# georgeretsi/smirk

Hardware: AMD Instinct MI355X
Metric: faces/sec (encode+FLAME+render+generate) @224x224 (higher is better)
Workload: dtype f32 results; encoder + generator convs as split-fp16 x3 MFMA with f32 accumulate (fp32-class error), FLAME / raster f32

## Files before the change

include/smirk_hip.h:

```cpp
#ifndef SMIRK_HIP_H
#define SMIRK_HIP_H

#include <stddef.h>
#include <stdint.h>

#ifdef __cplusplus
extern "C" {
#endif

#define SMIRK_OK 0
#define SMIRK_ERR_BAD_ARG (-1)
#define SMIRK_ERR_WORKSPACE (-2)
#define SMIRK_ERR_LAUNCH (-3)
#define SMIRK_ERR_UNSUPPORTED (-4)

const char* smirk_strerror(int code);
unsigned smirk_range_flag_peek(void);
void smirk_range_flag_clear(void);

int smirk_abi_version(void);

#define SMIRK_FLAME_KCHUNK 32

typedef struct SmirkFlameModel {
// ... 21 lines not shown
    const int32_t* dyn_faces;     const float* dyn_bary;
    const int32_t* full_faces;    const float* full_bary;
    const int32_t* mp_faces;      const float* mp_bary;
} SmirkFlameModel;

size_t smirk_flame_workspace_bytes(const SmirkFlameModel* m , int B);

int smirk_flame_forward(const SmirkFlameModel* m, int B,
                        const float* shape, int ns_in, const float* exp, int ne_in,
                        const float* global_pose , const float* neck , const float* jaw ,
                        const float* eye , const float* eyelid ,
                        float* verts, float* lmk_fan, float* lmk_fan3d, float* lmk_mp, int32_t* lut_idx_out,
                        float* v_posed_out, void* ws, size_t ws_bytes, void* stream);

size_t smirk_flame_backward_workspace_bytes(const SmirkFlameModel* m , int B);
int smirk_flame_backward(const SmirkFlameModel* m, const float* dirs_t, int B,
                         const float* shape, int ns_in, const float* exp, int ne_in,
                         const float* global_pose, const float* neck, const float* jaw, const float* eye, const float* eyelid,
                         const float* v_posed, const int32_t* lut_idx,
                         const float* g_verts, const float* g_lmk_fan, const float* g_lmk_fan3d, const float* g_lmk_mp,
                         float* d_shape, float* d_exp, float* d_global_pose, float* d_neck, float* d_jaw, float* d_eye, float* d_eyelid,
                         void* ws, size_t ws_bytes, void* stream);

int smirk_vertices2landmarks(const float* verts, int B, int V, const int32_t* faces ,
                             const int32_t* faces_idx, const float* bary, int L, float* out, void* stream);

typedef struct SmirkRenderMesh {
    int32_t V;
    int32_t Vf;
    int32_t Ff;
    int32_t nnz;
    const int32_t* keep;
    const int32_t* faces;
    const int32_t* nrm_ptr;
    const int32_t* nrm_face;
    const int32_t* nrm_corner;
} SmirkRenderMesh;

size_t smirk_render_workspace_bytes(const SmirkRenderMesh* mesh , int B, int H, int W);

int smirk_render_forward(const SmirkRenderMesh* mesh, int B, int H, int W,
                         const float* verts, const float* cam,
                         float* transformed, float* img,
                         int64_t* pix_to_face, float* bary, float* zbuf, float* normals,
                         void* ws, size_t ws_bytes, void* stream);

int smirk_vertex_normals(const SmirkRenderMesh* mesh, int B, const float* verts, float* normals, void* stream);

int smirk_project_landmarks(const float* lmk, const float* cam, int B, int L, float* out, void* stream);

size_t smirk_render_backward_workspace_bytes(const SmirkRenderMesh* mesh , int B, int H, int W);
int smirk_render_backward(const SmirkRenderMesh* mesh, int B, int H, int W,
                          const float* verts, const float* cam, const int64_t* pix_to_face,
                          const float* g_img, const float* g_transformed,
                          float* d_verts, float* d_cam, void* ws, size_t ws_bytes, void* stream);

int smirk_project_landmarks_backward(const float* lmk, const float* cam, const float* g_out, int B, int L,
                                     float* d_lmk, float* d_cam_accum, void* stream);

enum { SMIRK_PAD_ZERO = 0, SMIRK_PAD_REFLECT = 1 };
enum { SMIRK_ACT_NONE = 0, SMIRK_ACT_RELU = 1 };
enum { SMIRK_OUT_NHWC = 0, SMIRK_OUT_CONVT2X2 = 1 };

typedef struct SmirkConvDesc {
    int32_t B, H, W;
    int32_t C0, C1;
    int32_t Cout;
    int32_t KH, KW;
    int32_t stride;
    int32_t pad_t, pad_l;
    int32_t Ho, Wo;
    int32_t pad_mode;
    int32_t act;
    int32_t out_mode;
} SmirkConvDesc;

int smirk_conv_igemm_f32(const SmirkConvDesc* d, const float* in0, const float* in1, const float* w,
                         const float* scale, const float* shift, const float* residual, float* out, void* stream);

int smirk_conv_igemm_f16x3(const SmirkConvDesc* d, const void* in0, const void* in1, const void* w,
                           const float* scale, const float* shift, const void* residual, void* out, void* stream);
int smirk_conv_igemm_f16x1(const SmirkConvDesc* d, const void* in0, const void* in1, const void* w,
                           const float* scale, const float* shift, const void* residual, void* out, void* stream);
int smirk_conv3x3_tail_f16x3(const SmirkConvDesc* d, const void* in0, const void* in1, const void* w, const float* scale,
                             const float* shift, const float* fw, const float* fb, float* out_nchw, int fcout, void* stream);
int smirk_conv3x3_pool_f16x3(const SmirkConvDesc* d, const void* in0, const void* in1, const void* w, const float* scale, const float* shift, void* out,
                             void* pooled, void* stream);
int smirk_enc1_fused_supported(int cin_pad, int features, int H, int W);
int smirk_enc1_fused_split16(const void* x, const void* w1, const float* scale1, const float* shift1, const void* w2, const float* scale2,
                             const float* shift2, void* e1, void* pooled, int B, int H, int W, void* stream);
int smirk_f32_to_split16(const float* in, void* out, size_t n_elems, void* stream);
int smirk_split16_to_f32(const void* in, float* out, size_t n_elems, void* stream);
int smirk_split16_range_check(const void* in, size_t n_elems, float limit, uint32_t* counts, void* stream);
int smirk_maxpool2x2_split16(const void* in, void* out, int B, int H, int W, int C, void* stream);
int smirk_pack_generator_input_split16(const float* a, int Ca, const float* b, int Cb, void* out, int B, int H, int W, void* stream);
int smirk_conv1x1_sigmoid_nchw_split16(const void* in, const float* w , const float* bias, float* out,
                                       int B, int H, int W, int C, int Cout, void* stream);

int smirk_maxpool2x2_nhwc(const float* in, float* out, int B, int H, int W, int C, void* stream);
int smirk_nchw_to_nhwc_pad(const float* in, float* out, int B, int Cin, int H, int W, int Cpad, void* stream);
int smirk_pack_generator_input(const float* rendered, const float* masked, float* out, int B, int H, int W, void* stream);
int smirk_conv1x1_sigmoid_nchw(const float* in, const float* w , const float* bias, float* out,
                               int B, int H, int W, int C, int Cout, void* stream);

int smirk_stem_conv_s2(const float* img_nchw, const float* w , const float* scale,
                       const float* shift, float* out, int B, int H, int W, int Cout, void* stream);
int smirk_dwconv3x3(const float* in, const float* w , const float* scale, const float* shift, float* out,
                    int B, int H, int W, int C, int stride, int relu, void* stream);
int smirk_gap_linear(const float* feat, const float* w, const float* bias, float* out, float* ws, int B, int HW, int C, int N,
                     void* stream);
int smirk_stem_conv_s2_split16(const float* img_nchw, const float* w, const float* scale, const float* shift, void* out, int B, int H,
                               int W, int Cout, void* stream);
int smirk_dwconv3x3_split16(const void* in, const float* w , const float* scale, const float* shift, void* out, int B, int H,
                            int W, int C, int stride, int relu, void* stream);
int smirk_gap_linear_split16(const void* feat, const float* w, const float* bias, float* out, float* ws, int B, int HW, int C, int N,
                             void* stream);
int smirk_expression_clamps(float* params, int B, int n_exp, void* stream);

int smirk_mask_face_weights(const float* tverts, const float* normals, const int32_t* faces , const float* face_prob ,
                            int B, int V, int F, float* weights , void* stream);
int smirk_sample_faces(const float* weights, int B, int F, int num, uint64_t seed, uint64_t offset, int32_t* idx, float* bary,
                       void* stream);
int smirk_points_to_pixels(const float* points, int B, int L, int image_size, int64_t* out, void* stream);
int smirk_maxpool_sq(const float* in, float* tmp, float* out, int B, int H, int W, int radius, int complement, void* stream);
int smirk_bernoulli_field(float* out, size_t n, float p, uint64_t seed, uint64_t offset, void* stream);
int smirk_masking_compose(const float* img, const float* mask, const float* rendered_mask, const float* extra_points ,
                          const float* pmask ,
                          const float* keep, const float* noise_mult, int B, int C, int H, int W, int gen_noise,
                          uint64_t seed, uint64_t offset, float* out, void* stream);
int smirk_rendered_mask(const float* rendered_img, int B, int C, int H, int W, float* out, void* stream);
int smirk_scatter_points_mask(const int64_t* points, const int64_t* rbound, int B, int L, int H, int W, float* out, void* stream);
int smirk_transfer_pixels(const float* img, const int64_t* points1, const int64_t* points2, const int64_t* rbound, int B, int C,
                          int L, int H, int W, int32_t* winner_ws, float* out, void* stream);

size_t smirk_mbconv_lds_bytes(int Cin, int mid, int Cout, int stride);
int smirk_mbconv_image_supported(int H, int W, int Cin, int mid, int Cout, int stride);
int smirk_mbconv_image_split16(const void* x, const void* wexp, const float* s1, const float* b1, const float* wdw, const float* s2, const float* b2,
                               const void* wproj, const float* s3, const float* b3, int residual, void* out, int B, int H, int W, int Cin, int mid,
                               int Cout, void* stream);
int smirk_encoder_head_supported(int stem_cout, int kind, int cin, int mid, int cout, int stride, int skip);
int smirk_encoder_head_fused_split16(const float* img, const float* stem_w, const float* stem_scale, const float* stem_shift, const float* dw_w,
                                     const float* dw_scale, const float* dw_shift, const void* pw_w, const float* pw_scale, const float* pw_shift,
                                     int residual, void* out, int B, int H, int W, int stride, void* stream);
int smirk_mbconv_supported(int Cin, int mid, int Cout, int stride);
int smirk_mbconv_fused_split16(const void* x, const void* wexp, const float* s1, const float* b1, const float* wdw, const float* s2,
                               const float* b2, const void* wproj, const float* s3, const float* b3, int residual, void* out,
                               int B, int H, int W, int Cin, int mid, int Cout, int stride, void* stream);

typedef struct SmirkConvLayer {
    const void* w;
    const float* scale;
    const float* shift;
} SmirkConvLayer;

#define SMIRK_GEN_MAX_RES 16
enum { SMIRK_PRECISION_F32 = 0, SMIRK_PRECISION_F16X3 = 1 };

typedef struct SmirkGeneratorWeights {
    int32_t in_channels, out_channels, features, res_blocks;
    int32_t precision;
    int32_t cin_pad;
    SmirkConvLayer enc[5][2];
    SmirkConvLayer res[SMIRK_GEN_MAX_RES][2];
    SmirkConvLayer up[4];
    SmirkConvLayer dec[4][2];
    const float* final_w;
// ... 115 lines not shown
```

smirk_amd/_lib.py:

```python
import ctypes as C
import os

import torch

HERE = os.path.dirname(os.path.abspath(__file__))
LIB_PATH = os.path.join(HERE, "lib", "libsmirk_hip.so")
LIB_PATH = os.environ.get("SMIRK_HIP_LIBRARY", LIB_PATH)
ABI_VERSION = 12
PACK_DEPTHWISE, PACK_STEM, PACK_CONVT2X2 = -3, -27, -2
SMIRK_OK, SMIRK_ERR_BAD_ARG, SMIRK_ERR_WORKSPACE, SMIRK_ERR_LAUNCH, SMIRK_ERR_UNSUPPORTED = 0, -1, -2, -3, -4

_p = C.c_void_p
_i = C.c_int
_sz = C.c_size_t


class SmirkFlameModel(C.Structure):
    _fields_ = [(n, C.c_int32) for n in ("V", "VP", "F", "n_shape", "n_exp", "KP", "n_static", "n_dyn", "n_lut",
                                         "n_full", "n_mp", "_pad")] + \
               [(n, _p) for n in ("dirs", "v_template", "lbs_weights", "jdirs", "jtemplate", "l_eyelid", "r_eyelid",
                                  "faces", "static_faces", "static_bary", "dyn_faces", "dyn_bary", "full_faces",
                                  "full_bary", "mp_faces", "mp_bary")]


class SmirkRenderMesh(C.Structure):
    _fields_ = [(n, C.c_int32) for n in ("V", "Vf", "Ff", "nnz")] + \
               [(n, _p) for n in ("keep", "faces", "nrm_ptr", "nrm_face", "nrm_corner")]


class SmirkConvDesc(C.Structure):
    _fields_ = [(n, C.c_int32) for n in ("B", "H", "W", "C0", "C1", "Cout", "KH", "KW", "stride", "pad_t", "pad_l",
                                         "Ho", "Wo", "pad_mode", "act", "out_mode")]


class SmirkConvLayer(C.Structure):
    _fields_ = [("w", _p), ("scale", _p), ("shift", _p)]


GEN_MAX_RES, BACKBONE_MAX_BLOCKS = 16, 24
PRECISION_F32, PRECISION_F16X3 = 0, 1


class SmirkGeneratorWeights(C.Structure):
    _fields_ = [(n, C.c_int32) for n in ("in_channels", "out_channels", "features", "res_blocks", "precision", "cin_pad")] + \
               [("enc", SmirkConvLayer * 2 * 5), ("res", SmirkConvLayer * 2 * GEN_MAX_RES), ("up", SmirkConvLayer * 4),
                ("dec", SmirkConvLayer * 2 * 4), ("final_w", _p), ("final_b", _p)]


class SmirkMbBlock(C.Structure):
    _fields_ = [(n, C.c_int32) for n in ("kind", "stride", "cin", "mid", "cout", "skip")] + \
               [("pw", SmirkConvLayer), ("dw", SmirkConvLayer), ("pwl", SmirkConvLayer)]


class SmirkBackboneWeights(C.Structure):
    _fields_ = [(n, C.c_int32) for n in ("n_blocks", "precision", "n_out", "clamp_n_exp", "stem_cout", "feat_ch")] + \
               [("stem", SmirkConvLayer), ("blocks", SmirkMbBlock * BACKBONE_MAX_BLOCKS), ("head_w", _p), ("head_b", _p)]


class SmirkProfileRecord(C.Structure):
    _fields_ = [("kernel", C.c_char * 120), ("flop", C.c_double), ("bytes", C.c_double), ("ms", C.c_float), ("_pad", C.c_int32)]


PAD_ZERO, PAD_REFLECT = 0, 1
ACT_NONE, ACT_RELU = 0, 1
OUT_NHWC, OUT_CONVT2X2 = 0, 1

_SIGS = {
    "smirk_strerror": (C.c_char_p, [_i]),
    "smirk_abi_version": (_i, []),
    "smirk_range_flag_peek": (C.c_uint, []),
    "smirk_range_flag_clear": (None, []),
    "smirk_flame_workspace_bytes": (_sz, [C.POINTER(SmirkFlameModel), _i]),
    "smirk_flame_forward": (_i, [C.POINTER(SmirkFlameModel), _i, _p, _i, _p, _i, _p, _p, _p, _p, _p, _p, _p, _p, _p, _p,
                                 _p, _p, _sz, _p]),
    "smirk_flame_backward_workspace_bytes": (_sz, [C.POINTER(SmirkFlameModel), _i]),
    "smirk_flame_backward": (_i, [C.POINTER(SmirkFlameModel), _p, _i, _p, _i, _p, _i] + [_p] * 5 + [_p, _p] + [_p] * 4 + [_p] * 7 +
                             [_p, _sz, _p]),
    "smirk_vertices2landmarks": (_i, [_p, _i, _i, _p, _p, _p, _i, _p, _p]),
    "smirk_render_workspace_bytes": (_sz, [C.POINTER(SmirkRenderMesh), _i, _i, _i]),
    "smirk_render_forward": (_i, [C.POINTER(SmirkRenderMesh), _i, _i, _i, _p, _p, _p, _p, _p, _p, _p, _p, _p, _sz, _p]),
    "smirk_vertex_normals": (_i, [C.POINTER(SmirkRenderMesh), _i, _p, _p, _p]),
    "smirk_mask_face_weights": (_i, [_p, _p, _p, _p, _i, _i, _i, _p, _p]),
    "smirk_sample_faces": (_i, [_p, _i, _i, _i, C.c_uint64, C.c_uint64, _p, _p, _p]),
    "smirk_points_to_pixels": (_i, [_p, _i, _i, _i, _p, _p]),
    "smirk_maxpool_sq": (_i, [_p, _p, _p, _i, _i, _i, _i, _i, _p]),
    "smirk_bernoulli_field": (_i, [_p, _sz, C.c_float, C.c_uint64, C.c_uint64, _p]),
    "smirk_masking_compose": (_i, [_p, _p, _p, _p, _p, _p, _p, _i, _i, _i, _i, _i, C.c_uint64, C.c_uint64, _p, _p]),
    "smirk_render_backward_workspace_bytes": (_sz, [C.POINTER(SmirkRenderMesh), _i, _i, _i]),
    "smirk_render_backward": (_i, [C.POINTER(SmirkRenderMesh), _i, _i, _i, _p, _p, _p, _p, _p, _p, _p, _p, _sz, _p]),
    "smirk_project_landmarks_backward": (_i, [_p, _p, _p, _i, _i, _p, _p, _p]),
    "smirk_encoder_head_supported": (_i, [_i] * 7),
    "smirk_encoder_head_fused_split16": (_i, [_p] * 10 + [_i, _p] + [_i] * 4 + [_p]),
    "smirk_mbconv_image_supported": (_i, [_i] * 6),
    "smirk_mbconv_image_split16": (_i, [_p] * 10 + [_i, _p] + [_i] * 6 + [_p]),
    "smirk_mbconv_lds_bytes": (_sz, [_i, _i, _i, _i]),
    "smirk_mbconv_supported": (_i, [_i, _i, _i, _i]),
    "smirk_mbconv_fused_split16": (_i, [_p] * 10 + [_i, _p] + [_i] * 7 + [_p]),
    "smirk_warp_affine_u8": (_i, [_p, _i, _i, _i, _p, _i, _i, _i, _p, _p, _p]),
    "smirk_resize_linear_u8": (_i, [_p, _i, _i, _i, _i, _i, _i, _p, _p, _p]),
    "smirk_f32_nchw_to_u8_grid": (_i, [_p, _i, _i, _i, _i, _p, _i, _i, _p]),
    "smirk_u8_hwc_to_f32_nchw": (_i, [_p, _i, _i, _i, _i, _p, _p]),
    "smirk_interp_bilinear_f32": (_i, [_p, _i, _i, _i, _i, _i, _p, _p]),
    "smirk_hull_mask": (_i, [_p, _i, _i, _i, _i, _i, _p, _p]),
    "smirk_rendered_mask": (_i, [_p, _i, _i, _i, _i, _p, _p]),
    "smirk_scatter_points_mask": (_i, [_p, _p, _i, _i, _i, _i, _p, _p]),
    "smirk_transfer_pixels": (_i, [_p, _p, _p, _p, _i, _i, _i, _i, _i, _p, _p, _p]),
    "smirk_project_landmarks": (_i, [_p, _p, _i, _i, _p, _p]),
    "smirk_conv_igemm_f32": (_i, [C.POINTER(SmirkConvDesc), _p, _p, _p, _p, _p, _p, _p, _p]),
    "smirk_conv_igemm_f16x3": (_i, [C.POINTER(SmirkConvDesc), _p, _p, _p, _p, _p, _p, _p, _p]),
    "smirk_conv_igemm_f16x1": (_i, [C.POINTER(SmirkConvDesc), _p, _p, _p, _p, _p, _p, _p, _p]),
    "smirk_conv3x3_tail_f16x3": (_i, [C.POINTER(SmirkConvDesc), _p, _p, _p, _p, _p, _p, _p, _p, _i, _p]),
    "smirk_conv3x3_pool_f16x3": (_i, [C.POINTER(SmirkConvDesc), _p, _p, _p, _p, _p, _p, _p, _p]),
    "smirk_enc1_fused_supported": (_i, [_i, _i, _i, _i]),
    "smirk_enc1_fused_split16": (_i, [_p] * 9 + [_i, _i, _i, _p]),
    "smirk_f32_to_split16": (_i, [_p, _p, _sz, _p]),
    "smirk_split16_to_f32": (_i, [_p, _p, _sz, _p]),
    "smirk_maxpool2x2_split16": (_i, [_p, _p, _i, _i, _i, _i, _p]),
    "smirk_split16_range_check": (_i, [_p, _sz, C.c_float, _p, _p]),
    "smirk_pack_generator_input_split16": (_i, [_p, _i, _p, _i, _p, _i, _i, _i, _p]),
    "smirk_conv1x1_sigmoid_nchw_split16": (_i, [_p, _p, _p, _p, _i, _i, _i, _i, _i, _p]),
    "smirk_maxpool2x2_nhwc": (_i, [_p, _p, _i, _i, _i, _i, _p]),
    "smirk_nchw_to_nhwc_pad": (_i, [_p, _p, _i, _i, _i, _i, _i, _p]),
    "smirk_pack_generator_input": (_i, [_p, _p, _p, _i, _i, _i, _p]),
    "smirk_conv1x1_sigmoid_nchw": (_i, [_p, _p, _p, _p, _i, _i, _i, _i, _i, _p]),
    "smirk_stem_conv_s2": (_i, [_p, _p, _p, _p, _p, _i, _i, _i, _i, _p]),
    "smirk_dwconv3x3": (_i, [_p, _p, _p, _p, _p, _i, _i, _i, _i, _i, _i, _p]),
    "smirk_gap_linear": (_i, [_p, _p, _p, _p, _p, _i, _i, _i, _i, _p]),
    "smirk_stem_conv_s2_split16": (_i, [_p, _p, _p, _p, _p, _i, _i, _i, _i, _p]),
    "smirk_dwconv3x3_split16": (_i, [_p, _p, _p, _p, _p, _i, _i, _i, _i, _i, _i, _p]),
    "smirk_gap_linear_split16": (_i, [_p, _p, _p, _p, _p, _i, _i, _i, _i, _p]),
    "smirk_expression_clamps": (_i, [_p, _i, _i, _p]),
    "smirk_generator_workspace_bytes": (_sz, [C.POINTER(SmirkGeneratorWeights), _i, _i, _i]),
    "smirk_generator_forward": (_i, [C.POINTER(SmirkGeneratorWeights), _p, _i, _p, _i, _p, _i, _i, _i, C.POINTER(_p), _p, _sz, _p]),
    "smirk_backbone_workspace_bytes": (_sz, [C.POINTER(SmirkBackboneWeights), _i, _i, _i]),
    "smirk_backbone_forward": (_i, [C.POINTER(SmirkBackboneWeights), _p, _i, _i, _i, _p, _p, _p, _sz, _p]),
    "smirk_train_reduce_workspace_bytes": (_sz, [_i]),
    "smirk_conv_stats_rows_max": (_sz, [C.POINTER(SmirkConvDesc)]),
    "smirk_conv_igemm_stats_split16": (_i, [C.POINTER(SmirkConvDesc), _p, _p, _p, _p, _p, C.POINTER(C.c_int), _i, _p]),
    "smirk_bn_train_forward_partials_split16": (_i, [_p, _sz, _i, _p, _p, _p, _i, C.c_float, C.c_float, _p, _p, _p, _p, _p, _p, _p, _p, _i, _i, _p]),
    "smirk_dwconv3x3_stats_split16": (_i, [_p, _p, _p, _i, _i, _i, _i, _i, _p, C.POINTER(C.c_int), _p]),
    "smirk_bn_train_forward_split16": (_i, [_p, _sz, _i, _p, _p, _p, _i, C.c_float, C.c_float, _p, _p, _p, _p, _p, _p, _p, _p, _sz, _p]),
    "smirk_bn_train_backward_split16": (_i, [_p, _p, _sz, _i, _p, _p, _p, _p, _i, _p, _p, _p, _p, _sz, _p]),
    "smirk_bn_eval_forward_split16": (_i, [_p, _sz, _i, _p, _p, _p, _p, _p, _i, C.c_float, _p, _p, _p, _p]),
    "smirk_bn_eval_backward_split16": (_i, [_p, _p, _sz, _i, _p, _p, _p, _p, _p, _i, _p, _p]),
    "smirk_colsum_split16": (_i, [_p, _sz, _i, _p, _p, _sz, _p]),
    "smirk_maxpool2x2_backward_split16": (_i, [_p, _p, _p, _p, _i, _i, _i, _i, _p]),
    "smirk_reflect_pad1_backward_split16": (_i, [_p, _p, _p, _i, _i, _i, _i, _p]),
    "smirk_space_to_depth2_split16": (_i, [_p, _p, _i, _i, _i, _i, _p]),
    "smirk_conv1x1_sigmoid_backward_split16": (_i, [_p, _p, _p, _p, _p, _i, _i, _i, _i, _i, _p]),
    "smirk_conv_wgrad_set_mode": (_i, [_i]),
    "smirk_conv_wgrad_workspace_bytes": (_sz, [_i, _i, _i, _i, _i, _i]),
    "smirk_conv_wgrad_f32": (_i, [_p, _p, _p, _i, _i, _i, _i, _i, _i, _i, _p, _sz, _p]),
    "smirk_conv_wgrad_f16x1": (_i, [_p, _p, _p, _i, _i, _i, _i, _i, _i, _i, _p, _sz, _p]),
    "smirk_conv_wgrad_param": (_i, [_p, _p, _p, _i, _i, _i, _i, _i, _i, _i, _i, _i, _i, _i, _i, _p, _sz, _p]),
    "smirk_conv_wgrad_x1_fallbacks": (C.c_ulonglong, []),
    "smirk_pack_conv_weights_batch_split16": (_i, [_p, _i, C.c_ulonglong, _p]),
    "smirk_pack_conv_weights_split16": (_i, [_p, _i, _i, _i, _i, _i, _i, _p, _p, _p]),
    "smirk_stem_conv_s2_raw_split16": (_i, [_p, _p, _p, _i, _i, _i, _i, _p]),
    "smirk_stem_conv_s2_wgrad_workspace_bytes": (_sz, [_i]),
    "smirk_stem_conv_s2_wgrad_split16": (_i, [_p, _p, _p, _i, _i, _i, _i, _p, _sz, _p]),
    "smirk_stem_conv_s2_dgrad_split16": (_i, [_p, _p, _p, _i, _i, _i, _i, _p]),
    "smirk_dwconv3x3_dgrad_split16": (_i, [_p, _p, _p, _p, _i, _i, _i, _i, _i, _p]),
    "smirk_dwconv3x3_wgrad_workspace_bytes": (_sz, [_i]),
    "smirk_dwconv3x3_wgrad_split16": (_i, [_p, _p, _p, _i, _i, _i, _i, _i, _p, _sz, _p]),
    "smirk_dwconv3x3_wgrad_param_split16": (_i, [_p, _p, _p, _i, _i, _i, _i, _i, _p, _sz, _p]),
    "smirk_gap_linear_backward_split16": (_i, [_p, _p, _p, _p, _p, _p, _i, _i, _i, _i, _p]),
    "smirk_profile_start": (_i, []),
    "smirk_profile_stop": (_i, [C.POINTER(SmirkProfileRecord), _i]),
    "smirk_random_point_budget": (_i, [_p, _i, _i, C.c_float, C.c_uint64, C.c_uint64, _p]),
    "smirk_cycle_augment_workspace_bytes": (_sz, [_i]),
    "smirk_cycle_augment": (_i, [_p] * 6 + [_i] * 6 + [_p, _p, _p, _i, C.c_uint64, C.c_uint64] + [_p] * 6 + [_p, _p, _sz, _p]),
}
EXPORTS = tuple(_SIGS)

_LIB = None


class SmirkHipError(RuntimeError):
    pass


def lib():
    global _LIB
    if _LIB is None:
        if not os.path.exists(LIB_PATH):
            raise SmirkHipError(f"{LIB_PATH} not found: build it with `python -m smirk_amd.build` "
                                "(smirk_amd has no CPU / eager fallback)")
        L = C.CDLL(LIB_PATH)
        for name, (res, args) in _SIGS.items():
            fn = getattr(L, name)
            fn.restype, fn.argtypes = res, args
        if L.smirk_abi_version() != ABI_VERSION:
            raise SmirkHipError("libsmirk_hip.so ABI version mismatch; rebuild")
# ... 103 lines not shown
```

smirk_amd/csrc/capi.hip:

```cpp
#include <stdlib.h>
#include <string.h>

#include <map>
#include <mutex>
#include <utility>
#include <vector>

#include "common.h"

extern "C" const char* smirk_strerror(int code) {
    switch (code) {
        case SMIRK_OK: return "ok";
        case SMIRK_ERR_BAD_ARG: return "bad argument (null pointer, size or alignment constraint violated)";
        case SMIRK_ERR_WORKSPACE: return "workspace too small (see smirk_*_workspace_bytes)";
        case SMIRK_ERR_LAUNCH: return "HIP kernel launch failed";
        case SMIRK_ERR_UNSUPPORTED: return "configuration not supported by the gfx950 kernels";
        default: return "unknown smirk error";
    }
}

extern "C" int smirk_abi_version(void) { return 12; }

int smirk_switch(SmirkSwitch s) {
    static const char* const names[] = {"SMIRK_IGEMM_HALO", "SMIRK_IGEMM_PP", "SMIRK_CONV_RING", "SMIRK_DISABLE_PATCH_KERNEL", "SMIRK_DISABLE_ENC1_FUSED",
                                        "SMIRK_DISABLE_MBCONV_IMAGE", "SMIRK_DISABLE_MBCONV_TILE", "SMIRK_DISABLE_MBCONV_FUSED",
                                        "SMIRK_DISABLE_ENCODER_HEAD_FUSED", "SMIRK_GEN_SPLIT_CHAINS", "SMIRK_WGRAD_F16"};
    static_assert(sizeof(names) / sizeof(names[0]) == SMIRK_SW_COUNT, "one name per SmirkSwitch");
    const char* e = getenv(names[s]);
    switch (s) {
        case SMIRK_SW_IGEMM_HALO:
        case SMIRK_SW_CONV_RING: return !e || e[0] != '0';
        case SMIRK_SW_IGEMM_PP: return !e ? 1 : e[0] == '0' ? 0 : e[0] == 'a' ? 2 : 1;
        case SMIRK_SW_GEN_SPLIT_CHAINS: return !e ? 0 : e[0] == '0' ? 1 : e[0] == '3' ? 3 : 2;
        case SMIRK_SW_WGRAD_F16: return e ? atoi(e) : SMIRK_WGRAD_F16_DEFAULT;
        default: return e != nullptr;
    }
}

namespace {
std::mutex g_dev_mu;
std::map<std::pair<int, const void*>, size_t> g_lds_raised;
std::map<int, int> g_dev_cus;
}

int smirk_raise_dynamic_lds(const void* kernel, size_t bytes) {
    int dev = 0;
    if (hipGetDevice(&dev) != hipSuccess) { (void)hipGetLastError(); return SMIRK_ERR_LAUNCH; }
    std::lock_guard<std::mutex> lk(g_dev_mu);
    size_t& raised = g_lds_raised[{dev, kernel}];
    if (bytes <= raised) return SMIRK_OK;
    if (hipFuncSetAttribute(kernel, hipFuncAttributeMaxDynamicSharedMemorySize, (int)bytes) != hipSuccess) { (void)hipGetLastError(); return SMIRK_ERR_LAUNCH; }
    raised = bytes;
    return SMIRK_OK;
}

int smirk_device_cus() {
    int dev = 0;
    if (hipGetDevice(&dev) != hipSuccess) { (void)hipGetLastError(); return 256; }
    std::lock_guard<std::mutex> lk(g_dev_mu);
    auto it = g_dev_cus.find(dev);
    if (it != g_dev_cus.end()) return it->second;
    int cus = 0;
    if (hipDeviceGetAttribute(&cus, hipDeviceAttributeMultiprocessorCount, dev) != hipSuccess || cus <= 0) { (void)hipGetLastError(); cus = 256; }
    g_dev_cus[dev] = cus;
    return cus;
}

namespace {
std::once_flag g_range_once;
unsigned* g_range_host = nullptr;
unsigned* g_range_dev = nullptr;
}
unsigned* smirk_range_flag_device_ptr() {
    std::call_once(g_range_once, [] {
        void* h = nullptr;
        if (hipHostMalloc(&h, 64, hipHostMallocMapped | hipHostMallocPortable) != hipSuccess || !h) { (void)hipGetLastError(); return; }
        *(volatile unsigned*)h = 0u;
        void* d = nullptr;
        if (hipHostGetDevicePointer(&d, h, 0) != hipSuccess || !d) { (void)hipGetLastError(); (void)hipHostFree(h); return; }
        g_range_host = (unsigned*)h;
        g_range_dev = (unsigned*)d;
    });
    return g_range_dev;
}
extern "C" unsigned smirk_range_flag_peek(void) { return g_range_host ? *(volatile unsigned*)g_range_host : 0u; }
extern "C" void smirk_range_flag_clear(void) { if (g_range_host) *(volatile unsigned*)g_range_host = 0u; }

bool g_smirk_prof_on = false;
namespace {
struct ProfRec { char name[120]; double flop, bytes; hipEvent_t e0, e1; };
std::vector<ProfRec> g_recs;
std::mutex g_prof_mu;
thread_local char t_next_name[120];
thread_local double t_next_flop = 0.0, t_next_bytes = 0.0;
thread_local bool t_has_name = false;
thread_local long t_open = -1;
}

void smirk_prof_next(const char* name, double flop, double bytes) {
    if (!g_smirk_prof_on) return;
    t_has_name = name != nullptr;
    if (name) { strncpy(t_next_name, name, sizeof(t_next_name) - 1); t_next_name[sizeof(t_next_name) - 1] = 0; }
    t_next_flop = flop; t_next_bytes = bytes;
}
// ... 55 lines not shown
```

smirk_amd/csrc/conv.hip:

```cpp
#include <stdio.h>
#include <stdlib.h>

#include "common.h"
#include <type_traits>

#include "conv_common.h"

__device__ __attribute__((aligned(16))) float g_zero16_conv[4] = {0.f, 0.f, 0.f, 0.f};
#define g_zero16 g_zero16_conv

__device__ __forceinline__ const float* psel(bool c, const float* p, const float* q) {
    const unsigned long long m = 0ull - (unsigned long long)c;
    return (const float*)(((unsigned long long)p & m) | ((unsigned long long)q & ~m));
}

enum { KW_GENERIC = 0, KW_FAST = 1, KW_FAST_KT = 2, KW_CMAJOR = 3, KW_LEAN = 4, KW_LEAN_CM = 5 };

template <int BM, int BN, int WGM, int WGN, bool SPLIT, int KWALK, bool X1 = false, bool STATS = false>
__device__ __forceinline__ void conv_tile(const ConvArgs& a, float* smem, const int m0, const int n0) {
    constexpr int NW = WGM * WGN, NT = 64 * NW;
    constexpr int RP = NT / 8;
    constexpr int TM = BM / WGM / 32, TN = BN / WGN / 32;
    constexpr int PA = BM / RP, PB = BN / RP;
    constexpr int STAGE = (BM + BN) * 32;
// ... 480 lines not shown
                    float v = acc[0][i][j][r] * sc + sh;
                    size_t o;
                    int b, y, x;
                    row_to_pixel(m, HoWo, d.Wo, a.psh, b, y, x);
                    if (convt) o = (((size_t)b * 2 * d.Ho + 2 * y + dy) * 2 * d.Wo + 2 * x + dx) * d.Cout + co;
                    else o = (((size_t)b * d.Ho + y) * d.Wo + x) * d.Cout + n;
                    if (a.residual) v += a.residual[o];
                    if (d.act == SMIRK_ACT_RELU) v = fmaxf(v, 0.f);
                    a.out[o] = v;
                }
            }
        }
    }
}

template <int BM, int BN, int WGM, int WGN, bool SPLIT, int KWALK, bool X1 = false, bool STATS = false>
__global__ __launch_bounds__(64 * WGM * WGN, 2) void conv_igemm_kernel(ConvArgs a) {
    __shared__ __attribute__((aligned(16))) float smem[2 * (BM + BN) * 32];
    const int ntn = (a.N + BN - 1) / BN;
    const int logical = xcd_logical(blockIdx.x, gridDim.x);
    const int mt = logical / ntn, nt = logical % ntn;
    conv_tile<BM, BN, WGM, WGN, SPLIT, KWALK, X1, STATS>(a, smem, mt * BM, nt * BN);
}

template <int BM, int BN, int WGM, int WGN, bool SPLIT, int KWALK, bool X1 = false>
static void launch_igemm_kw(const ConvArgs& a, hipStream_t st) {
    const int ntm = (a.M + BM - 1) / BM, ntn = (a.N + BN - 1) / BN;
    if (g_smirk_prof_on) {
        char nm[120];
        snprintf(nm, sizeof(nm), "conv_igemm_kernel<%d,%d,%d,%d,%s,%d>%s", BM, BN, WGM, WGN, SPLIT ? "true" : "false", KWALK, X1 ? "[f16x1]" : "");
        const double px = (double)a.d.B * a.d.H * a.d.W;
        smirk_prof_next(nm, 2.0 * a.M * a.N * a.K, 4.0 * (px * a.Cin + (double)a.M * a.N + (double)a.N * a.K + (a.residual ? (double)a.M * a.N : 0.0)));
    }
    if constexpr (SPLIT && (KWALK == KW_LEAN || KWALK == KW_LEAN_CM || KWALK == KW_FAST_KT)) {
        if (a.stats) {
            SMIRK_LAUNCH((conv_igemm_kernel<BM, BN, WGM, WGN, SPLIT, KWALK, X1, true>), dim3(ntm * ntn), dim3(64 * WGM * WGN), 0, st, a);
            return;
        }
    }
    SMIRK_LAUNCH((conv_igemm_kernel<BM, BN, WGM, WGN, SPLIT, KWALK, X1>), dim3(ntm * ntn), dim3(64 * WGM * WGN), 0, st, a);
}

template <int BM, int BN, int WGM, int WGN, bool SPLIT, bool X1 = false>
static void launch_igemm(const ConvArgs& a, hipStream_t st) {
    const SmirkConvDesc& d = a.d;
    const bool lean = true;
    if constexpr (SPLIT && WGM * WGN == 4) {
        const long long b0 = (long long)d.B * d.H * d.W * d.C0 * 4, b1 = (long long)d.B * d.H * d.W * d.C1 * 4, bw = (long long)a.N * a.K * 4;
        if (lean && (d.C0 % CV_BK == 0) && (d.C1 % CV_BK == 0) && b0 < (1ll << 31) && b1 < (1ll << 31) && bw < (1ll << 31)) {
            const bool pow2 = (d.C0 & (d.C0 - 1)) == 0 && (d.C1 & (d.C1 - 1)) == 0, even = ((d.C0 + d.C1) / CV_BK) % 2 == 0;
            const bool want_cm = BN == 128;
            if (want_cm && d.KH == 3 && d.KW == 3 && pow2 && even) launch_igemm_kw<BM, BN, WGM, WGN, SPLIT, KW_LEAN_CM, X1>(a, st);
            else launch_igemm_kw<BM, BN, WGM, WGN, SPLIT, KW_LEAN, X1>(a, st);
            return;
        }
    }
    const bool cmajor = BN == 128 && d.Ho * d.Wo >= 400;
    if constexpr (SPLIT && WGM * WGN == 4) {
        if (cmajor && d.KH == 3 && d.KW == 3 && (d.C0 % CV_BK == 0) && (d.C1 % CV_BK == 0)) {
            launch_igemm_kw<BM, BN, WGM, WGN, SPLIT, KW_CMAJOR, X1>(a, st);
            return;
        }
    }
    if ((d.C0 % CV_BK == 0) && (d.C1 % CV_BK == 0)) launch_igemm_kw<BM, BN, WGM, WGN, SPLIT, KW_FAST, X1>(a, st);
    else if (d.KH * d.KW == 1) launch_igemm_kw<BM, BN, WGM, WGN, SPLIT, KW_FAST_KT, X1>(a, st);
    else launch_igemm_kw<BM, BN, WGM, WGN, SPLIT, KW_GENERIC, X1>(a, st);
}

bool smirk_conv_pp_eligible(const ConvArgs& a);
int smirk_conv_pp_launch(const ConvArgs& a, hipStream_t st);

bool smirk_conv_halo_eligible(const ConvArgs& a);
int smirk_conv_halo_launch(const ConvArgs& a, hipStream_t st, bool x1);

bool smirk_conv3x3_patch_eligible(const SmirkConvDesc* d, bool has_residual);
int smirk_conv3x3_patch_launch(const SmirkConvDesc* d, const void* in0, const void* in1, const void* w, const float* scale,
                               const float* shift, void* out, hipStream_t st, const float* fw, const float* fb, float* fout,
                               int fcout);

bool smirk_conv3x3_ring64_eligible(const SmirkConvDesc* d, bool has_residual);
int smirk_conv3x3_ring64_launch(const SmirkConvDesc* d, const void* in0, const void* in1, const void* w, const float* scale, const float* shift, void* out,
                                void* pooled, hipStream_t st, float* stats = nullptr, int* stats_rows = nullptr);

static int conv_dispatch_one(const SmirkConvDesc* d, const void* in0, const void* in1, const void* w, const float* scale,
                             const float* shift, const void* residual, void* out, void* stream, bool split, bool x1 = false, float* stats = nullptr,
                             int* stats_rows = nullptr);

static int conv_batch_chunk(const SmirkConvDesc* d, bool split) {
    if (!split || d->B <= 1) return d->B;
    const long long px = (long long)d->H * d->W, per = 4 * px * (d->C0 > d->C1 ? d->C0 : d->C1), lim = (1ll << 31) - 1;
    if (per * d->B <= lim || per > lim) return d->B;
    return (int)(lim / per);
}

static int conv_dispatch(const SmirkConvDesc* d, const void* in0, const void* in1, const void* w, const float* scale,
                         const float* shift, const void* residual, void* out, void* stream, bool split, bool x1 = false, float* stats = nullptr,
                         int* stats_rows = nullptr) {
    if (!d || !in0 || !w || !out) return SMIRK_ERR_BAD_ARG;
    if (stats_rows) *stats_rows = 0;
    const int bc = (d->B > 0 && d->H > 0 && d->W > 0 && d->C0 > 0 && d->C1 >= 0) ? conv_batch_chunk(d, split) : d->B;
    if (bc >= d->B) return conv_dispatch_one(d, in0, in1, w, scale, shift, residual, out, stream, split, x1, stats, stats_rows);
    const size_t ipx = (size_t)d->H * d->W, opx = (size_t)d->Ho * d->Wo * (d->out_mode == SMIRK_OUT_CONVT2X2 ? 4 : 1);
    for (int b0 = 0; b0 < d->B; b0 += bc) {
        SmirkConvDesc dc = *d;
        dc.B = d->B - b0 < bc ? d->B - b0 : bc;
        const int rc = conv_dispatch_one(&dc, (const float*)in0 + b0 * ipx * d->C0, in1 ? (const float*)in1 + b0 * ipx * d->C1 : nullptr, w, scale, shift,
                                         residual ? (const float*)residual + b0 * opx * d->Cout : nullptr, (float*)out + b0 * opx * d->Cout, stream, split, x1);
        if (rc != SMIRK_OK) return rc;
    }
    return SMIRK_OK;
}

static int conv_dispatch_one(const SmirkConvDesc* d, const void* in0, const void* in1, const void* w, const float* scale,
                             const float* shift, const void* residual, void* out, void* stream, bool split, bool x1, float* stats, int* stats_rows) {
    if (!d || !in0 || !w || !out) return SMIRK_ERR_BAD_ARG;
    if (stats_rows) *stats_rows = 0;
    if (x1 && !split) return SMIRK_ERR_BAD_ARG;
    const int cq = split ? 8 : 4;
    if (d->B <= 0 || d->H <= 0 || d->W <= 0 || d->Cout <= 0 || d->C0 <= 0 || d->C0 % cq || d->C1 % cq || d->C1 < 0 ||
        (d->C1 > 0 && !in1) || d->Ho <= 0 || d->Wo <= 0 || d->stride <= 0 || (split && d->Cout % 8))
        return SMIRK_ERR_BAD_ARG;
    if (!((d->KH == 3 && d->KW == 3) || (d->KH == 1 && d->KW == 1))) return SMIRK_ERR_UNSUPPORTED;
    if (d->pad_mode == SMIRK_PAD_REFLECT && (d->H < 2 || d->W < 2 || d->pad_t > 1 || d->pad_l > 1)) return SMIRK_ERR_UNSUPPORTED;
    ConvArgs a;
    a.d = *d; a.in0 = (const float*)in0; a.in1 = (const float*)in1; a.w = (const float*)w; a.scale = scale; a.shift = shift;
    a.residual = (const float*)residual; a.out = (float*)out;
    a.Cin = d->C0 + d->C1;
    a.K = d->KH * d->KW * a.Cin;
    a.N = d->Cout;
    if (d->out_mode == SMIRK_OUT_CONVT2X2) {
        if (d->KH != 1 || d->C1 != 0 || d->Ho != d->H || d->Wo != d->W || d->stride != 1 || residual) return SMIRK_ERR_UNSUPPORTED;
        a.N = 4 * d->Cout;
    }
    const long long M = (long long)d->B * d->Ho * d->Wo;
    if (M > (1ll << 30) || (long long)d->B * d->H * d->W > (1ll << 30)) return SMIRK_ERR_UNSUPPORTED;
    a.M = (int)M;
    a.stats = nullptr;
    a.psh = 0;
    if (d->KH == 3)
        while (a.psh < 4 && d->Ho % (2 << a.psh) == 0 && d->Wo % (2 << a.psh) == 0) ++a.psh;
    hipStream_t st = (hipStream_t)stream;
    const bool no_patch = smirk_switch(SMIRK_SW_DISABLE_PATCH_KERNEL);
    if (split && !x1 && !no_patch && smirk_conv3x3_ring64_eligible(d, residual != nullptr))
        return smirk_conv3x3_ring64_launch(d, in0, in1, w, scale, shift, out, nullptr, st, stats, stats_rows);
    if (split && !x1 && !no_patch && smirk_conv3x3_patch_eligible(d, residual != nullptr))
        return smirk_conv3x3_patch_launch(d, in0, in1, w, scale, shift, out, st, nullptr, nullptr, nullptr, 0);
    const bool want_stats = split && stats && stats_rows && d->out_mode == SMIRK_OUT_NHWC && !scale && !shift && !residual && d->act == SMIRK_ACT_NONE;
    if (split && smirk_conv_halo_eligible(a)) {
        if (want_stats) { a.stats = stats; *stats_rows = ((a.M + 255) / 256) * 4; }
        return smirk_conv_halo_launch(a, st, x1);
    }
    if (split && !x1 && smirk_conv_pp_eligible(a)) return smirk_conv_pp_launch(a, st);
    if (want_stats) {
        const long long b0 = (long long)d->B * d->H * d->W * d->C0 * 4, b1 = (long long)d->B * d->H * d->W * d->C1 * 4, bw = (long long)a.N * a.K * 4;
        const bool lean = (d->C0 % CV_BK == 0) && (d->C1 % CV_BK == 0) && b0 < (1ll << 31) && b1 < (1ll << 31) && bw < (1ll << 31);
        const bool kt = !((d->C0 % CV_BK == 0) && (d->C1 % CV_BK == 0)) && d->KH * d->KW == 1;
        if (lean || kt) {
            const int BMt = a.N > 32 ? 128 : 256, WGMt = a.N > 32 ? 2 : 4;
            a.stats = stats;
            *stats_rows = ((a.M + BMt - 1) / BMt) * WGMt;
        }
    }
    if (split && x1) {
        if (a.N > 64) launch_igemm<128, 128, 2, 2, true, true>(a, st);
        else if (a.N > 32) launch_igemm<128, 64, 2, 2, true, true>(a, st);
        else launch_igemm<256, 32, 4, 1, true, true>(a, st);
    } else if (split) {
        if (a.N > 64) launch_igemm<128, 128, 2, 2, true>(a, st);
        else if (a.N > 32) launch_igemm<128, 64, 2, 2, true>(a, st);
        else launch_igemm<256, 32, 4, 1, true>(a, st);
    } else {
        if (a.N > 64) launch_igemm<128, 128, 2, 2, false>(a, st);
        else if (a.N > 32) launch_igemm<128, 64, 2, 2, false>(a, st);
        else launch_igemm<256, 32, 4, 1, false>(a, st);
    }
    return smirk_launch_status();
}

extern "C" int smirk_conv_igemm_f32(const SmirkConvDesc* d, const float* in0, const float* in1, const float* w,
                                    const float* scale, const float* shift, const float* residual, float* out,
                                    void* stream) {
    return conv_dispatch(d, in0, in1, w, scale, shift, residual, out, stream, false);
}

extern "C" int smirk_conv3x3_pool_f16x3(const SmirkConvDesc* d, const void* in0, const void* in1, const void* w, const float* scale, const float* shift, void* out,
                                        void* pooled, void* stream) {
    if (!d || !in0 || !w || !out || !pooled) return SMIRK_ERR_BAD_ARG;
    if (d->C0 % 8 || d->C1 % 8 || (d->C1 > 0 && !in1) || d->H % 2 || d->W % 2) return SMIRK_ERR_BAD_ARG;
    if (d->B <= 0 || d->H <= 0 || d->W <= 0 || d->C0 <= 0) return SMIRK_ERR_BAD_ARG;
    const int bc = conv_batch_chunk(d, true);
    if (bc <= 0) return SMIRK_ERR_UNSUPPORTED;
    {
        SmirkConvDesc d0 = *d;
        d0.B = d->B < bc ? d->B : bc;
        if (d0.Cout != 64 || !smirk_conv3x3_ring64_eligible(&d0, false)) return SMIRK_ERR_UNSUPPORTED;
    }
    const size_t px = (size_t)d->H * d->W;
    for (int b0 = 0; b0 < d->B; b0 += bc) {
        SmirkConvDesc dc = *d;
        dc.B = d->B - b0 < bc ? d->B - b0 : bc;
        const int rc = smirk_conv3x3_ring64_launch(&dc, (const float*)in0 + b0 * px * d->C0, in1 ? (const float*)in1 + b0 * px * d->C1 : nullptr, w, scale, shift,
                                                   (float*)out + b0 * px * d->Cout, (float*)pooled + b0 * (px / 4) * d->Cout, (hipStream_t)stream);
        if (rc != SMIRK_OK) return rc;
    }
    return SMIRK_OK;
}

extern "C" int smirk_conv3x3_tail_f16x3(const SmirkConvDesc* d, const void* in0, const void* in1, const void* w, const float* scale,
                                        const float* shift, const float* fw, const float* fb, float* out_nchw, int fcout,
                                        void* stream) {
    if (!d || !in0 || !w || !fw || !out_nchw || fcout <= 0 || fcout > 4 || d->Cout != 32) return SMIRK_ERR_BAD_ARG;
    if (d->C0 % 8 || d->C1 % 8 || (d->C1 > 0 && !in1) || d->act != SMIRK_ACT_RELU) return SMIRK_ERR_BAD_ARG;
    if (!smirk_conv3x3_patch_eligible(d, false)) return SMIRK_ERR_UNSUPPORTED;
    const int bc = (d->B > 0 && d->H > 0 && d->W > 0 && d->C0 > 0 && d->C1 >= 0) ? conv_batch_chunk(d, true) : d->B;
    if (bc >= d->B) return smirk_conv3x3_patch_launch(d, in0, in1, w, scale, shift, nullptr, (hipStream_t)stream, fw, fb, out_nchw, fcout);
    const size_t px = (size_t)d->H * d->W;
    for (int b0 = 0; b0 < d->B; b0 += bc) {
        SmirkConvDesc dc = *d;
        dc.B = d->B - b0 < bc ? d->B - b0 : bc;
        const int rc = smirk_conv3x3_patch_launch(&dc, (const float*)in0 + b0 * px * d->C0, in1 ? (const float*)in1 + b0 * px * d->C1 : nullptr, w, scale, shift,
                                                  nullptr, (hipStream_t)stream, fw, fb, out_nchw + b0 * px * fcout, fcout);
        if (rc != SMIRK_OK) return rc;
    }
    return SMIRK_OK;
}

extern "C" int smirk_conv_igemm_f16x3(const SmirkConvDesc* d, const void* in0, const void* in1, const void* w,
                                      const float* scale, const float* shift, const void* residual, void* out,
                                      void* stream) {
    return conv_dispatch(d, in0, in1, w, scale, shift, residual, out, stream, true);
}

extern "C" int smirk_conv_igemm_f16x1(const SmirkConvDesc* d, const void* in0, const void* in1, const void* w,
                                      const float* scale, const float* shift, const void* residual, void* out,
                                      void* stream) {
// ... 285 lines not shown
```

Before: 10370.

## Add streaming 1x1 conv kernel for small-Cin wide-Cout expansions

Adds a dedicated 1x1 convolution kernel that stages a 64-row activation tile in LDS once and streams over all output-channel tiles, reading weights directly from global memory and computing the split-fp16 products with 32x32x16 MFMA. It is dispatched for NHWC 1x1 convs with C0<=64, Cout>=6*C0 and small spatial maps, targeting expansion convs where the generic igemm tiling wastes work or launches poorly. The per-tile accumulator goes through an LDS transpose buffer for a coalesced epilogue with scale/shift/relu. It adds a new code path whose behaviour under the split precision scheme must match the existing kernels.

```diff
diff --git a/include/smirk_hip.h b/include/smirk_hip.h
--- a/include/smirk_hip.h
+++ b/include/smirk_hip.h
@@ -127,6 +127,7 @@
                            const float* scale, const float* shift, const void* residual, void* out, void* stream);
 int smirk_conv_igemm_f16x1(const SmirkConvDesc* d, const void* in0, const void* in1, const void* w,
                            const float* scale, const float* shift, const void* residual, void* out, void* stream);
+int smirk_conv1x1_stream_eligible(const SmirkConvDesc* d, int has_residual);
 int smirk_conv3x3_tail_f16x3(const SmirkConvDesc* d, const void* in0, const void* in1, const void* w, const float* scale,
                              const float* shift, const float* fw, const float* fb, float* out_nchw, int fcout, void* stream);
 int smirk_conv3x3_pool_f16x3(const SmirkConvDesc* d, const void* in0, const void* in1, const void* w, const float* scale, const float* shift, void* out,
diff --git a/smirk_amd/_lib.py b/smirk_amd/_lib.py
--- a/smirk_amd/_lib.py
+++ b/smirk_amd/_lib.py
@@ -6,7 +6,7 @@
 HERE = os.path.dirname(os.path.abspath(__file__))
 LIB_PATH = os.path.join(HERE, "lib", "libsmirk_hip.so")
 LIB_PATH = os.environ.get("SMIRK_HIP_LIBRARY", LIB_PATH)
-ABI_VERSION = 12
+ABI_VERSION = 13
 PACK_DEPTHWISE, PACK_STEM, PACK_CONVT2X2 = -3, -27, -2
 SMIRK_OK, SMIRK_ERR_BAD_ARG, SMIRK_ERR_WORKSPACE, SMIRK_ERR_LAUNCH, SMIRK_ERR_UNSUPPORTED = 0, -1, -2, -3, -4
 
@@ -109,6 +109,7 @@
     "smirk_conv_igemm_f32": (_i, [C.POINTER(SmirkConvDesc), _p, _p, _p, _p, _p, _p, _p, _p]),
     "smirk_conv_igemm_f16x3": (_i, [C.POINTER(SmirkConvDesc), _p, _p, _p, _p, _p, _p, _p, _p]),
     "smirk_conv_igemm_f16x1": (_i, [C.POINTER(SmirkConvDesc), _p, _p, _p, _p, _p, _p, _p, _p]),
+    "smirk_conv1x1_stream_eligible": (_i, [C.POINTER(SmirkConvDesc), _i]),
     "smirk_conv3x3_tail_f16x3": (_i, [C.POINTER(SmirkConvDesc), _p, _p, _p, _p, _p, _p, _p, _p, _i, _p]),
     "smirk_conv3x3_pool_f16x3": (_i, [C.POINTER(SmirkConvDesc), _p, _p, _p, _p, _p, _p, _p, _p]),
     "smirk_enc1_fused_supported": (_i, [_i, _i, _i, _i]),
diff --git a/smirk_amd/csrc/capi.hip b/smirk_amd/csrc/capi.hip
--- a/smirk_amd/csrc/capi.hip
+++ b/smirk_amd/csrc/capi.hip
@@ -19,7 +19,7 @@
     }
 }
 
-extern "C" int smirk_abi_version(void) { return 12; }
+extern "C" int smirk_abi_version(void) { return 13; }
 
 int smirk_switch(SmirkSwitch s) {
     static const char* const names[] = {"SMIRK_IGEMM_HALO", "SMIRK_IGEMM_PP", "SMIRK_CONV_RING", "SMIRK_DISABLE_PATCH_KERNEL", "SMIRK_DISABLE_ENC1_FUSED",
diff --git a/smirk_amd/csrc/conv.hip b/smirk_amd/csrc/conv.hip
--- a/smirk_amd/csrc/conv.hip
+++ b/smirk_amd/csrc/conv.hip
@@ -586,6 +586,9 @@
 int smirk_conv3x3_ring64_launch(const SmirkConvDesc* d, const void* in0, const void* in1, const void* w, const float* scale, const float* shift, void* out,
                                 void* pooled, hipStream_t st, float* stats = nullptr, int* stats_rows = nullptr);
 
+extern "C" int smirk_conv1x1_stream_eligible(const SmirkConvDesc* d, int has_residual);
+int smirk_conv1x1_stream_launch(const ConvArgs& a, hipStream_t st);
+
 static int conv_dispatch_one(const SmirkConvDesc* d, const void* in0, const void* in1, const void* w, const float* scale,
                              const float* shift, const void* residual, void* out, void* stream, bool split, bool x1 = false, float* stats = nullptr,
                              int* stats_rows = nullptr);
@@ -655,6 +658,7 @@
         return smirk_conv_halo_launch(a, st, x1);
     }
     if (split && !x1 && smirk_conv_pp_eligible(a)) return smirk_conv_pp_launch(a, st);
+    if (split && !x1 && !stats && !no_patch && smirk_conv1x1_stream_eligible(d, residual != nullptr)) return smirk_conv1x1_stream_launch(a, st);
     if (want_stats) {
         const long long b0 = (long long)d->B * d->H * d->W * d->C0 * 4, b1 = (long long)d->B * d->H * d->W * d->C1 * 4, bw = (long long)a.N * a.K * 4;
         const bool lean = (d->C0 % CV_BK == 0) && (d->C1 % CV_BK == 0) && b0 < (1ll << 31) && b1 < (1ll << 31) && bw < (1ll << 31);
diff --git a/smirk_amd/csrc/conv_stream1x1.hip b/smirk_amd/csrc/conv_stream1x1.hip
--- /dev/null
+++ b/smirk_amd/csrc/conv_stream1x1.hip
@@ -0,0 +1,183 @@
+#include <stdio.h>
+
+#include "common.h"
+#include "conv_common.h"
+
+struct S1Args {
+    const float *in, *w, *scale, *shift;
+    float* out;
+    int M, N, K, Cout, H, W;
+    int ksteps, pitch;
+    int convt, relu;
+};
+
+#define S1_ROWS 64
+#define S1_TB (32 * 36)
+
+template <int KG, int NW>
+__global__ __launch_bounds__(64 * NW, KG <= 2 ? 3 : 2) void conv1x1_stream_kernel(S1Args a) {
+    constexpr int NT = 64 * NW;
+    extern __shared__ __attribute__((aligned(16))) char smem[];
+    const int tid = threadIdx.x, lane = tid & 63, fr = lane & 31, hb = lane >> 5;
+    const int wave = __builtin_amdgcn_readfirstlane(tid >> 6);
+    char* As = smem;
+    float* tb = (float*)(smem + S1_ROWS * a.pitch) + wave * S1_TB;
+    const int m0 = blockIdx.x * S1_ROWS;
+    const int nunits = 2 * ((a.N + 31) / 32);
+    const half8 hz = {0, 0, 0, 0, 0, 0, 0, 0};
+
+    auto load_b = [&](int u, int j, half8 (*dst)[2]) {
+        const int n = (u >> 1) * 32 + fr;
+        const bool nv = u < nunits && n < a.N;
+        const float* wrow = a.w + (size_t)(nv ? n : 0) * a.K;
+#pragma unroll
+        for (int s = 0; s < 4; ++s) {
+            const int g = 2 * (4 * j + s) + hb, gc = min(g, a.K / 8 - 1);
+            const bool v = nv && g * 8 < a.K;
+            const half8 t0 = *(const half8*)(wrow + gc * 8), t1 = *(const half8*)(wrow + gc * 8 + 4);
+            dst[s][0] = v ? t0 : hz;
+            dst[s][1] = v ? t1 : hz;
+        }
+    };
+    half8 bn[4][2];
+    load_b(wave, 0, bn);
+
+    {
+        constexpr int NIT = S1_ROWS * KG * 16 / NT;
+        const int P = a.ksteps * 4, Preal = a.K / 4;
+        f32x4 xv[NIT];
+#pragma unroll
+        for (int it = 0; it < NIT; ++it) {
+            const int idx = tid + NT * it, row = idx / P, pc = idx - row * P;
+            const bool in = idx < S1_ROWS * P && m0 + row < a.M && pc < Preal;
+            const f32x4 t = *(const f32x4*)(a.in + (size_t)min(m0 + row, a.M - 1) * a.K + min(pc, Preal - 1) * 4);
+            const f32x4 z = {0.f, 0.f, 0.f, 0.f};
+            xv[it] = in ? t : z;
+        }
+#pragma unroll
+        for (int it = 0; it < NIT; ++it) {
+            const int idx = tid + NT * it, row = idx / P, pc = idx - row * P;
+            if (idx < S1_ROWS * P) *(f32x4*)(As + row * a.pitch + pc * 16) = xv[it];
+        }
+    }
+    asm volatile("s_waitcnt lgkmcnt(0)" ::: "memory");
+    __builtin_amdgcn_s_barrier();
+    asm volatile("" ::: "memory");
+
+    SmirkRangeAcc rng;
+    const int HW = a.H * a.W;
+    for (int u = wave; u < nunits; u += NW) {
+        const int rb = u & 1, n0 = (u >> 1) * 32;
+        const int ng = n0 + (lane & 3) * 8;
+        const bool gv = ng < a.N;
+        const int co = a.convt ? ng % a.Cout : ng, coc = gv ? co : 0;
+        f32x4 sc0 = {1.f, 1.f, 1.f, 1.f}, sc1 = sc0, sh0 = {0.f, 0.f, 0.f, 0.f}, sh1 = sh0;
+        if (a.scale) { sc0 = *(const f32x4*)(a.scale + coc); sc1 = *(const f32x4*)(a.scale + coc + 4); }
+        if (a.shift) { sh0 = *(const f32x4*)(a.shift + coc); sh1 = *(const f32x4*)(a.shift + coc + 4); }
+
+        f32x16 acc0, acc1;
+#pragma unroll
+        for (int r = 0; r < 16; ++r) { acc0[r] = 0.f; acc1[r] = 0.f; }
+        const char* arow = As + (rb * 32 + fr) * a.pitch + hb * 32;
+#pragma unroll
+        for (int j = 0; j < KG; ++j) {
+            half8 bc[4][2];
+#pragma unroll
+            for (int s = 0; s < 4; ++s) { bc[s][0] = bn[s][0]; bc[s][1] = bn[s][1]; }
+            if (j + 1 < KG) load_b(u, j + 1, bn); else load_b(u + NW, 0, bn);
+#pragma unroll
+            for (int s = 0; s < 4; ++s) {
+                const int S = 4 * j + s;
+                if (S < a.ksteps) {
+                    const half8 ah = *(const half8*)(arow + S * 64), al = *(const half8*)(arow + S * 64 + 16);
+                    acc0 = __builtin_amdgcn_mfma_f32_32x32x16_f16(ah, bc[s][0], acc0, 0, 0, 0);
+                    acc1 = __builtin_amdgcn_mfma_f32_32x32x16_f16(ah, bc[s][1], acc1, 0, 0, 0);
+                    acc1 = __builtin_amdgcn_mfma_f32_32x32x16_f16(al, bc[s][0], acc1, 0, 0, 0);
+                }
+            }
+        }
+
+#pragma unroll
+        for (int r = 0; r < 16; ++r) tb[mfma32_row(r, lane) * 36 + fr] = __builtin_fmaf(acc1[r], 1.0f / 2048.0f, acc0[r]);
+        asm volatile("s_waitcnt lgkmcnt(0)" ::: "memory");
+#pragma unroll
+        for (int it = 0; it < 2; ++it) {
+            const int row = (it * 64 + lane) >> 2, m = m0 + rb * 32 + row;
+            if (m < a.M && gv) {
+                float v[8];
+                *(f32x4*)v = *(const f32x4*)(tb + row * 36 + (lane & 3) * 8);
+                *(f32x4*)(v + 4) = *(const f32x4*)(tb + row * 36 + (lane & 3) * 8 + 4);
+                size_t o;
+                if (a.convt) {
+                    const int b = m / HW, rem = m - b * HW, y = rem / a.W, x = rem - y * a.W;
+                    const int q = ng / a.Cout, dy = q >> 1, dx = q & 1;
+                    o = (((size_t)b * 2 * a.H + 2 * y + dy) * 2 * a.W + 2 * x + dx) * a.Cout + co;
+                } else {
+                    o = (size_t)m * a.Cout + ng;
+                }
+                if (a.scale) {
+#pragma clang fp contract(off)
+#pragma unroll
+                    for (int q = 0; q < 4; ++q) { v[q] *= sc0[q]; v[4 + q] *= sc1[q]; }
+                }
+                if (a.shift) {
+#pragma clang fp contract(off)
+#pragma unroll
+                    for (int q = 0; q < 4; ++q) { v[q] += sh0[q]; v[4 + q] += sh1[q]; }
+                }
+                if (a.relu) {
+#pragma unroll
+                    for (int q = 0; q < 8; ++q) v[q] = fmaxf(v[q], 0.f);
+                }
+                half8 hi, lo;
+                split8(v, hi, lo, rng);
+                *(half8*)(a.out + o) = hi;
+                *(half8*)(a.out + o + 4) = lo;
+            }
+        }
+        asm volatile("s_waitcnt lgkmcnt(0)" ::: "memory");
+    }
+    rng.commit();
+}
+
+static bool stream_eligible(const SmirkConvDesc* d, bool has_residual) {
+    if (!d || has_residual) return false;
+    if (d->KH != 1 || d->KW != 1 || d->stride != 1 || d->C1 != 0 || d->pad_t != 0 || d->pad_l != 0) return false;
+    if (d->B <= 0 || d->H <= 0 || d->W <= 0 || d->Ho != d->H || d->Wo != d->W) return false;
+    if (d->C0 <= 0 || d->C0 % 8 || d->Cout <= 0 || d->Cout % 8 || d->C0 > 256) return false;
+    if (d->out_mode != SMIRK_OUT_NHWC && d->out_mode != SMIRK_OUT_CONVT2X2) return false;
+    return d->out_mode == SMIRK_OUT_NHWC && d->C0 <= 64 && d->Cout >= 6 * d->C0 && d->H * d->W <= 256;
+}
+
+extern "C" int smirk_conv1x1_stream_eligible(const SmirkConvDesc* d, int has_residual) { return stream_eligible(d, has_residual != 0) ? 1 : 0; }
+
+template <int KG, int NW>
+static int stream_launch(const S1Args& a, hipStream_t st) {
+    const size_t lds = (size_t)S1_ROWS * a.pitch + (size_t)NW * S1_TB * 4;
+    const int rc = smirk_raise_dynamic_lds((const void*)conv1x1_stream_kernel<KG, NW>, lds);
+    if (rc != SMIRK_OK) return rc;
+    if (g_smirk_prof_on) {
+        char nm[64];
+        snprintf(nm, sizeof(nm), "conv1x1_stream_kernel<%d,%d>%s", KG, NW, a.convt ? "[convT]" : "");
+        smirk_prof_next(nm, 2.0 * a.M * a.N * a.K, 4.0 * ((double)a.M * a.K + (double)a.M * a.N + (double)a.N * a.K));
+    }
+    SMIRK_LAUNCH((conv1x1_stream_kernel<KG, NW>), dim3((a.M + S1_ROWS - 1) / S1_ROWS), dim3(64 * NW), lds, st, a);
+    return smirk_launch_status();
+}
+
+int smirk_conv1x1_stream_launch(const ConvArgs& c, hipStream_t st) {
+    if (!stream_eligible(&c.d, c.residual != nullptr)) return SMIRK_ERR_UNSUPPORTED;
+    S1Args a;
+    a.in = c.in0; a.w = c.w; a.scale = c.scale; a.shift = c.shift; a.out = c.out;
+    a.M = c.M; a.N = c.N; a.K = c.K; a.Cout = c.d.Cout; a.H = c.d.H; a.W = c.d.W;
+    a.ksteps = (c.K + 15) / 16;
+    a.pitch = a.ksteps * 64 + 16;
+    a.convt = c.d.out_mode == SMIRK_OUT_CONVT2X2;
+    a.relu = c.d.act == SMIRK_ACT_RELU;
+    switch ((a.ksteps + 3) / 4) {
+        case 1: return stream_launch<1, 4>(a, st);
+        case 2: return stream_launch<2, 4>(a, st);
+        case 3: return stream_launch<3, 4>(a, st);
+        default: return stream_launch<4, 8>(a, st);
+    }
+}
```

Result: no change. 10340 (-0.3%).
